# mfigura/Resilient-consensus-based-MARL

Measured on AMD Instinct MI355X. Metric: agent-steps/sec (whole RPBCAC training loop; + consensus-updates/sec), higher is better.
Workload: dtype f32 (matrix-core operands as 2 x f16 pieces: each fp32 operand to <= 1 ulp; the 20-unit layers run 3 of the 4 piece products)

## Files before the change

include/rcmarl.h:

```cpp
#ifndef RCMARL_H
#define RCMARL_H

#ifdef __cplusplus
extern "C" {
#endif

#define RCMARL_OK 0
#define RCMARL_ERR_ARG 1
#define RCMARL_ERR_LAUNCH 2
#define RCMARL_ERR_UNSUPPORTED 3

int rcmarl_abi_version(void);
int rcmarl_mb_job_layout(int what);
int rcmarl_fit_partial_size(int hid);
int rcmarl_actor_partial_size(int hid, int n_actions);
int rcmarl_rows_per_chunk(void);

int rcmarl_consensus_params(const float* msg, float* theta, const int* nbr, const int* coop, int S, int N,
                            int ldp, int P_hid, int d, int H, float* lo_dbg, float* hi_dbg, void* stream);
int rcmarl_consensus_params_circulant_supported(int N, int d, int H);
int rcmarl_consensus_params_circulant(const float* msg, float* theta, const int* coop, int S, int N, int ldp, int P_hid,
                                      int d, int H, float* lo_dbg, float* hi_dbg, void* stream);

typedef struct rcmarl_ragged_class {
// ... 28 lines not shown
                           void* stream);
int rcmarl_lattice_pack_dz_rowsum(const float* dz, void* dzp, float* sums, int sums_ld, int sums_off, int S, int N, int B, int hid,
                                  int ldb, int dzp_rt, int dzp_kt, void* stream);
int rcmarl_layer1_forward_lattice(const void* kp, int kp_rt, int kp_kt, const void* wp, int wp_rt, int wp_kt,
                                  const float* theta, float* a1t, int S, int N, int B, int in_dim, int hid, int ldp,
                                  int ldb, void* stream);
int rcmarl_layer1_backward_sgd_lattice(const void* ktp, int ktp_rt, int ktp_kt, const void* dzp, int dzp_rt, int dzp_kt,
                                       const float* alpha, float* theta, const int* mask, int S, int N, int B,
                                       int in_dim, int hid, int ldp, float lr, void* wp_out, int wp_rt, int wp_kt,
                                       void* stream);
int rcmarl_layer1_backward_sgd_lattice_tiled(const void* ktp, int ktp_rt, int ktp_kt, const void* dzp, int dzp_rt, int dzp_kt,
                                             const float* alpha, float* theta, const int* mask, int S, int N, int B,
                                             int in_dim, int hid, int ldp, float lr, void* wp_out, int wp_rt, int wp_kt,
                                             float* w_tiled, long w_tiled_bytes, int src_tiled, int dst_tiled, void* stream);
long rcmarl_lattice_w1_tiled_bytes(int S, int N, int in_dim, int hid);
int rcmarl_mid_fit_lattice(const float* a1t, const float* theta, const float* y, float* partials, void* dzp, int dzp_rt,
                           int dzp_kt, int S, int N, int B, int in_dim, int hid, int ldp, int ldb, int* ovf_flags, void* stream);


int rcmarl_shuffle_perms(const void* seeds, const int* calls, int n, int epochs, int B, int* perm, int S, void* stream);

int rcmarl_small_sgd(const float* partials, float* theta, const int* mask, float* loss_out, int S, int N,
                     int B, int in_dim, int hid, int ldp, float lr, void* stream);
int rcmarl_mid_value(const float* a1t, const float* theta, const float* r_applied, float gamma, float* out, int S,
                     int N, int B, int in_dim, int hid, int ldp, int ldb, void* stream);
int rcmarl_mid_value_f32(const float* a1t, const float* theta, const float* r_applied, float gamma, float* out, int S,
                         int N, int B, int in_dim, int hid, int ldp, int ldb, void* stream);

int rcmarl_consensus_head(const float* a1t, const float* theta, const float* msg, const int* nbr,
                          const int* coop, float* partials, float* agg_out, int S, int N, int B, int in_dim,
                          int hid, int ldp, int ldb, int d, int H, void* stream);
int rcmarl_consensus_head_ragged(const float* a1t, const float* theta, const float* msg, const int* nbr_off,
                                 const int* nbr_idx, const int* order, const rcmarl_ragged_class* classes, int n_classes,
                                 float* partials, float* agg_out, int S, int N, int B, int in_dim, int hid, int ldp, int ldb,
                                 void* stream);
int rcmarl_projection_residual(const float* a1t, const float* theta, const float* agg, const int* coop,
                               float* partials, int S, int N, int B, int in_dim, int hid, int ldp, int ldb,
                               void* stream);
int rcmarl_head_apply(const float* partials, float* theta, const int* coop, int S, int N, int B, int in_dim,
                      int hid, int ldp, void* stream);

int rcmarl_mid_actor(float* a1t, const float* theta, const float* act_t, const float* delta, float* partials, int S,
                     int N, int B, int in_dim, int hid, int n_actions, int ldp, int ldb, void* stream);
int rcmarl_small_adam(const float* partials, float* theta, float* adam_m, float* adam_v, const int* mask,
                      float* loss_out, int S, int N, int B, int in_dim, int hid, int n_actions, int ldp, float alpha,
                      float one_m_b1, float one_m_b2, float eps, void* stream);
// ... 164 lines not shown
```

resilient-consensus-based-marl_amd/capi.py:

```python
import ctypes as C
import os

c_f32p = C.c_void_p
c_i32p = C.c_void_p
c_u8p = C.c_void_p


class MbJob(C.Structure):
    _fields_ = [("x", C.c_void_p), ("x_seed_stride", C.c_long), ("theta", C.c_void_p), ("agents", C.c_void_p), ("n_adv", C.c_int),
                ("in_dim", C.c_int), ("ldp", C.c_int), ("reserved_", C.c_int), ("y", C.c_void_p), ("perm", C.c_void_p),
                ("loss_out", C.c_void_p), ("ovf_flags", C.c_void_p)]


class RaggedClass(C.Structure):
    _fields_ = [("d", C.c_int), ("H", C.c_int), ("first", C.c_int), ("count", C.c_int)]


c_f64p = C.c_void_p
c_stream = C.c_void_p

c_long = C.c_long
c_int = C.c_int
c_float = C.c_float

# ... 24 lines not shown
    "rcmarl_layer1_forward": [c_f32p, c_long, c_f32p, c_f32p, c_int, c_int, c_int, c_int, c_int, c_int, c_int,
                              c_stream],
    "rcmarl_layer1_backward_sgd": [c_f32p, c_long, c_f32p, c_f32p, c_u8p, c_int, c_int, c_int, c_int, c_int, c_int,
                                   c_int, c_float, c_stream],
    "rcmarl_layer1_backward_adam": [c_f32p, c_long, c_f32p, c_f32p, c_f32p, c_f32p, c_u8p, c_int, c_int, c_int, c_int,
                                    c_int, c_int, c_int, c_float, c_float, c_float, c_float, c_stream],
    "rcmarl_mid_fit": [c_f32p, c_f32p, c_f32p, c_f32p, c_int, c_int, c_int, c_int, c_int, c_int, c_int, c_stream],
    "rcmarl_lattice_encode": [c_f32p, c_long, c_f32p, c_int, c_int, c_int, c_u8p, c_int, c_int, c_u8p, c_int, c_int,
                              c_i32p, c_stream],
    "rcmarl_w1_split": [c_f32p, c_f32p, c_u8p, c_int, c_int, c_int, c_int, c_int, c_int, c_int, c_stream],
    "rcmarl_lattice_pack_dz": [c_f32p, c_u8p, c_int, c_int, c_int, c_int, c_int, c_int, c_int, c_stream],
    "rcmarl_lattice_pack_dz_rowsum": [c_f32p, c_u8p, c_f32p, c_int, c_int, c_int, c_int, c_int, c_int, c_int, c_int, c_int, c_stream],
    "rcmarl_layer1_forward_lattice": [c_u8p, c_int, c_int, c_u8p, c_int, c_int, c_f32p, c_f32p, c_int, c_int, c_int,
                                      c_int, c_int, c_int, c_int, c_stream],
    "rcmarl_layer1_backward_sgd_lattice": [c_u8p, c_int, c_int, c_u8p, c_int, c_int, c_f32p, c_f32p, c_u8p, c_int,
                                           c_int, c_int, c_int, c_int, c_int, c_float, c_u8p, c_int, c_int, c_stream],
    "rcmarl_layer1_backward_sgd_lattice_tiled": [c_u8p, c_int, c_int, c_u8p, c_int, c_int, c_f32p, c_f32p, c_u8p, c_int,
                                                 c_int, c_int, c_int, c_int, c_int, c_float, c_u8p, c_int, c_int, c_f32p, c_long,
                                                 c_int, c_int, c_stream],
    "rcmarl_mid_fit_lattice": [c_f32p, c_f32p, c_f32p, c_f32p, c_u8p, c_int, c_int, c_int, c_int, c_int, c_int, c_int,
                               c_int, c_int, c_i32p, c_stream],
    "rcmarl_shuffle_perms": [C.c_void_p, c_i32p, c_int, c_int, c_int, c_i32p, c_int, c_stream],
    "rcmarl_small_sgd": [c_f32p, c_f32p, c_u8p, c_f32p, c_int, c_int, c_int, c_int, c_int, c_int, c_float, c_stream],
    "rcmarl_mid_value": [c_f32p, c_f32p, c_f32p, c_float, c_f32p, c_int, c_int, c_int, c_int, c_int, c_int, c_int,
                         c_stream],
    "rcmarl_mid_value_f32": [c_f32p, c_f32p, c_f32p, c_float, c_f32p, c_int, c_int, c_int, c_int, c_int, c_int, c_int,
                             c_stream],
    "rcmarl_consensus_head": [c_f32p, c_f32p, c_f32p, c_i32p, c_u8p, c_f32p, c_f32p, c_int, c_int, c_int, c_int, c_int,
                              c_int, c_int, c_int, c_int, c_stream],
    "rcmarl_head_apply": [c_f32p, c_f32p, c_u8p, c_int, c_int, c_int, c_int, c_int, c_int, c_stream],
    "rcmarl_mid_actor": [c_f32p, c_f32p, c_f32p, c_f32p, c_f32p, c_int, c_int, c_int, c_int, c_int, c_int, c_int,
                         c_int, c_stream],
    "rcmarl_small_adam": [c_f32p, c_f32p, c_f32p, c_f32p, c_u8p, c_f32p, c_int, c_int, c_int, c_int, c_int, c_int,
                          c_int, c_float, c_float, c_float, c_float, c_stream],
    "rcmarl_team_reward": [c_f32p, c_long, c_u8p, c_int, c_f32p, c_int, c_int, c_int, c_int, c_stream],
    "rcmarl_projection_residual": [c_f32p, c_f32p, c_f32p, c_i32p, c_f32p, c_int, c_int, c_int, c_int, c_int, c_int,
                                   c_int, c_stream],
    "rcmarl_minibatch_fit": [c_f32p, c_long, c_f32p, c_i32p, c_int, c_f32p, c_i32p, c_int, c_int, c_int, c_int, c_int,
                             c_int, c_int, c_int, c_int, c_float, c_f32p, c_i32p, c_stream],
    "rcmarl_minibatch_actor": [c_f32p, c_long, c_f32p, c_f32p, c_f32p, c_i32p, c_int, c_f32p, c_f32p, c_i32p, c_int,
                               c_int, c_int, c_int, c_int, c_int, c_int, c_int, c_int, c_int, C.c_double, C.c_double,
                               C.c_double, C.c_double, c_int, c_f32p, c_stream],
    "rcmarl_minibatch_actor_wide_supported": [c_int, c_int, c_int, c_int],
    "rcmarl_minibatch_actor_wide": [c_f32p, c_long, c_f32p, c_f32p, c_f32p, c_f32p, c_i32p, c_int, c_f32p, c_f32p, c_i32p, c_int,
                                    c_int, c_int, c_int, c_int, c_int, c_int, c_int, c_int, c_int, C.c_double, C.c_double,
                                    C.c_double, C.c_double, c_int, c_f32p, c_stream],
# ... 145 lines not shown
```

resilient-consensus-based-marl_amd/csrc/lattice_gemm.hip:

```cpp
#include "rcmarl_lattice.h"
#include "rcmarl_lat_mainloop.h"
#include <type_traits>
#include <stdlib.h>

namespace {

__device__ __forceinline__ unsigned pack2(unsigned lo, unsigned hi) { return (lo & 0xffffu) | (hi << 16); }

__global__ __launch_bounds__(256) void k_lattice_encode(const float* __restrict__ x, long x_seed_stride,
                                                        const float* __restrict__ alpha, int B, int in_dim,
                                                        unsigned char* __restrict__ kp, int kp_rt, int kp_kt,
                                                        unsigned char* __restrict__ ktp, int ktp_rt, int ktp_kt,
                                                        int* __restrict__ flag, int kp_f16, int ktp_f16) {
  __shared__ unsigned short tileB[32][128 + 2], tileH[32][128 + 2];
  const int s = blockIdx.z, b0 = blockIdx.y * 32, c0 = blockIdx.x * 128;
  const int t = threadIdx.x;
  {
    const int cl = t & 127, c = c0 + cl;
    const float al = c < in_dim ? alpha[c] : 1.f;
    bool bad = false;
#pragma unroll 4
    for (int i = 0; i < 16; ++i) {
      const int bl = (t >> 7) + 2 * i, b = b0 + bl;
      float kq = 0.f;
// ... 160 lines not shown

struct LatPkOut {
  unsigned char* a1_bk; int bk_rt;
  unsigned char* a1_kb; int kb_kt;
  unsigned* s1; int s1_ld;
  int* ovf;
};

template <bool W8, bool F16, bool PK = false>
__global__ RC_LAT_OCC(W8 ? 512 : 256, W8 ? 4 : 2)
void k_lat_forward(const unsigned char* __restrict__ wp, int wp_rt, int wp_kt, const unsigned char* __restrict__ kp, int kp_rt,
                   int kp_kt, const float* __restrict__ theta, float* __restrict__ a1t, int S, int N, int B, int in_dim, int ldp,
                   int ldb, int mtiles, int ntiles, int hid, const LatPkOut pk) {
  constexpr int PA = F16 ? 2 : 3, PB = 1, MT = 2, NT = W8 ? 2 : 4, WM = 2, WN = W8 ? 4 : 2;
  typedef LatCfg<PA, PB, MT, NT, WM, WN> C;
  RCMARL_DYN_SMEM(unsigned char, lds);
  int s, w;
  lat_decode(blockIdx.x, mtiles * ntiles, S, s, w);
  const int bn = w % ntiles, bm = w / ntiles;
  LatOperands op;
  op.a = wp + (long)s * wp_rt * wp_kt * (PA * RC_PK_BLOCK); op.a_kt = wp_kt; op.art0 = bm * C::ART;
  op.b = kp + (long)s * kp_rt * kp_kt * (PB * RC_PK_BLOCK); op.b_kt = kp_kt; op.brt0 = bn * C::BRT;
  rc_f32x16 acc[MT][NT];
  lat_mainloop<PA, PB, MT, NT, WM, WN, false, F16>(op, (in_dim + 31) >> 5, lds, acc);
  const int ncols = N * hid;
  const float* theta_s = theta + (long)s * N * ldp;
  float* a1t_s = a1t + (long)s * ncols * ldb;
  __syncthreads();
  float* bias = reinterpret_cast<float*>(lds);
  if (threadIdx.x < C::BM) {
    const int col = bm * C::BM + threadIdx.x;
    const int ag = col / hid;
    bias[threadIdx.x] = col < ncols ? theta_s[(long)ag * ldp + in_dim * hid + (col - ag * hid)] : 0.f;
  }
  __syncthreads();
  const int lane = threadIdx.x & 63, half = lane >> 5;
  const int wave = __builtin_amdgcn_readfirstlane((int)(threadIdx.x >> 6)), wm = wave / WN, wn = wave % WN;
  float bv[MT][16];
#pragma unroll
  for (int mt = 0; mt < MT; ++mt)
#pragma unroll
    for (int q = 0; q < 4; ++q) {
      const float4 b4 = *reinterpret_cast<const float4*>(bias + wm * 32 * MT + 32 * mt + 8 * q + 4 * half);
      bv[mt][4 * q] = b4.x; bv[mt][4 * q + 1] = b4.y; bv[mt][4 * q + 2] = b4.z; bv[mt][4 * q + 3] = b4.w;
    }
  if constexpr (PK) {
    static_assert(F16, "packed activations exist in the two-piece f16 form");
// ... 428 lines not shown
```

resilient-consensus-based-marl_amd/csrc/mid_kernels.hip:

```cpp
#include "rcmarl_lattice.h"
#include <stdlib.h>
#include "selnet_generated.inc"

namespace {

constexpr bool kMidDropLL = true;

constexpr int ROWS = 256;
constexpr int LDR = ROWS + 1;

template <int HID> struct FitPart {
  static constexpr int gW2 = 0, gb2 = HID * HID, gW3 = gb2 + HID, gb3 = gW3 + HID, gb1 = gb3 + 1, loss = gb1 + HID,
                       SIZE = loss + 1, NSMALL = SIZE - gb2;
};
template <int HID, int A> struct ActorPart {
  static constexpr int gW2 = 0, gW3 = HID * HID, gb2 = gW3 + HID * A, gb3 = gb2 + HID, gb1 = gb3 + A,
                       loss = gb1 + HID, SIZE = loss + 1, NSMALL = SIZE - gb2;
};

template <int HID>
__device__ __forceinline__ void load_a1(const float* __restrict__ a1t, long row0, int ldb, int b, bool valid,
                                        float (&a1)[HID]) {
#pragma unroll
  for (int j = 0; j < HID; ++j) a1[j] = valid ? a1t[(row0 + j) * ldb + b] : 0.f;
// ... 541 lines not shown
#pragma unroll
        for (int u = 0; u < LU; ++u) {
          sRec[PT::gb1 + v8_unit(half, u)] = sm[u];
          sRec[PT::gW3 + v8_unit(half, u)] = sm[LU + u];
        }
        if (half == 0) { sRec[PT::gb3] = sm[2 * LU]; sRec[PT::loss] = sm[2 * LU + 1]; }
      }
    }
  }
  __syncthreads();
  if (amax > RC_V8_RANGE) ovf_flags[s * N + i] = ovf_gen;
  {
    const float* r0 = reinterpret_cast<const float*>(sPn + 0 * PANEL_B + 2 * PLANE * 2);
    const float* r1 = reinterpret_cast<const float*>(sPn + 1 * PANEL_B + 2 * PLANE * 2);
    const float* r2 = reinterpret_cast<const float*>(sPn + 2 * PANEL_B + 2 * PLANE * 2);
    const float* r3 = reinterpret_cast<const float*>(sPn + 3 * PANEL_B + 2 * PLANE * 2);
    float* out = partials + (((long)s * N + i) * gridDim.x + blockIdx.x) * PT::SIZE;
    out[r] = (r0[r] + r1[r]) + (r2[r] + r3[r]);
    if (r + ROWS < PT::SIZE) out[r + ROWS] = (r0[r + ROWS] + r1[r + ROWS]) + (r2[r + ROWS] + r3[r + ROWS]);
  }
}

template <int HID>
__global__ __launch_bounds__(256) void k_small_sgd(const float* __restrict__ partials, float* __restrict__ theta,
                                                   const int* __restrict__ mask,
                                                   float* __restrict__ loss_out, int N, int B, int in_dim, int ldp,
                                                   int nchunk, float lr) {
  typedef FitPart<HID> PT;
  const int s = blockIdx.y, i = blockIdx.x;
  if (mask && !mask[i]) return;
  const NetGeom g = make_geom(in_dim, HID, 1);
  float* th = theta + ((long)s * N + i) * ldp;
  const float* pp = partials + ((long)s * N + i) * nchunk * PT::SIZE;
  for (int e = threadIdx.x; e < PT::SIZE; e += blockDim.x) {
    float sum = 0.f;
    for (int c = 0; c < nchunk; ++c) sum += pp[(long)c * PT::SIZE + e];
    if (e == PT::loss) {
      if (loss_out) loss_out[(long)s * N + i] = sum / (float)B;
      continue;
    }
    int o;
    if (e < PT::gb2) o = g.o_W2 + e;
    else if (e < PT::gW3) o = g.o_b2 + (e - PT::gb2);
    else if (e < PT::gb3) o = g.o_W3 + (e - PT::gW3);
    else if (e < PT::gb1) o = g.o_b3;
    else o = g.o_b1 + (e - PT::gb1);
    th[o] = th[o] - lr * sum;
  }
}

template <int HID>
__global__ __launch_bounds__(256) void k_mid_value(const float* __restrict__ a1t, const float* __restrict__ theta,
                                                   const float* __restrict__ r_applied, float gamma,
                                                   float* __restrict__ out, int N, int B, int in_dim, int ldp,
                                                   int ldb) {
  const int s = blockIdx.z, i = blockIdx.y;
  const int b = blockIdx.x * ROWS + threadIdx.x;
  const bool valid = b < B;
  const NetGeom g = make_geom(in_dim, HID, 1);
  const float* th = theta + ((long)s * N + i) * ldp;
  float a1[HID], a2[HID];
  load_a1<HID>(a1t, ((long)s * N + i) * HID, ldb, b, valid, a1);
  layer2<HID>(th, g, a1, a2);
  const float v = head1<HID>(th + g.o_W3, th[g.o_b3], a2);
  if (valid) {
    const long o = ((long)s * N + i) * ldb + b;
    out[o] = r_applied ? r_applied[o] + gamma * v : v;
  }
}

// ... 761 lines not shown
  const dim3 grid(rc_ceil_div(nchunk, cpw), N, S), block(ROWS);
  rc_form_set(dzp, (rc_lat_f16_mode() >> 1) & 1);
  if (midfit_v8() && ovf_flags != nullptr) {
    int* flags = ovf_flags;
    int* gen = ovf_flags + (size_t)S * N;
    RCMARL_LAUNCH(k_bump_generation, dim3(1), dim3(1), 0, stream, gen);
    RC_HID_SWITCH(hid, RCMARL_LAUNCH((k_mid_fit_v8<HID_, true>), grid, block, 0, stream, const_cast<float*>(a1t), theta, y,
                                     partials, N, B, in_dim, ldp, ldb, nchunk, cpw, (unsigned char*)dzp, dzp_rt, dzp_kt, flags, (const int*)gen));
    RC_HID_SWITCH(hid, RCMARL_LAUNCH((k_mid_fit_v5<HID_, true, true>), grid, block, 0, stream, const_cast<float*>(a1t), theta, y,
                                     partials, N, B, in_dim, ldp, ldb, nchunk, cpw, (unsigned char*)dzp, dzp_rt, dzp_kt,
                                     (const int*)flags, (const int*)gen));
  } else if (rc_lat_f16_mode() & 2) {
    RC_HID_SWITCH(hid, RCMARL_LAUNCH((k_mid_fit_v5<HID_, true, true>), grid, block, 0, stream, const_cast<float*>(a1t), theta, y,
                                     partials, N, B, in_dim, ldp, ldb, nchunk, cpw, (unsigned char*)dzp, dzp_rt, dzp_kt,
                                     (const int*)nullptr, (const int*)nullptr));
  } else {
    RC_HID_SWITCH(hid, RCMARL_LAUNCH((k_mid_fit_v5<HID_, true>), grid, block, 0, stream, const_cast<float*>(a1t), theta, y,
                                     partials, N, B, in_dim, ldp, ldb, nchunk, cpw, (unsigned char*)dzp, dzp_rt, dzp_kt,
                                     (const int*)nullptr, (const int*)nullptr));
  }
  return rcmarl_check_launch();
}

RCMARL_EXPORT int rcmarl_small_sgd(const float* partials, float* theta, const int* mask, float* loss_out,
                                   int S, int N, int B, int in_dim, int hid, int ldp, float lr, void* stream) {
  if (!partials || !theta || S <= 0 || N <= 0 || B <= 0) return RCMARL_ERR_ARG;
  const int nchunk = rc_ceil_div(B, ROWS), nrec = rc_ceil_div(nchunk, midfit_cpw(nchunk, (long)S * N));
  const dim3 grid(N, S), block(256);
  RC_HID_SWITCH(hid, RCMARL_LAUNCH((k_small_sgd<HID_>), grid, block, 0, stream, partials, theta, mask, loss_out, N, B,
                                   in_dim, ldp, nrec, lr));
  return rcmarl_check_launch();
}

static int mid_value_impl(const float* a1t, const float* theta, const float* r_applied, float gamma, float* out, int S, int N, int B,
                          int in_dim, int hid, int ldp, int ldb, void* stream, bool f32_only) {
  if (bad_mid(a1t, theta, S, N, B, in_dim, hid, ldp, ldb) || !out) return RCMARL_ERR_ARG;
  const dim3 grid(rc_ceil_div(B, ROWS), N, S), block(ROWS);
  const char* mxe = getenv("RCMARL_MIDVALUE_MX");
  if (!f32_only && hid == 20 && !(mxe && atoi(mxe) == 0) && rc_lat_f16_mode() != 0) {
    const int nchunk = rc_ceil_div(B, ROWS);
    const long pairs = (long)N * S;
    int wgs = pairs >= 2048 ? 2 : (pairs >= 512 ? 4 : nchunk);
    if (wgs * 32 < nchunk) wgs = (nchunk + 31) / 32;
    const int cpw = (nchunk + wgs - 1) / wgs;
    const dim3 gmx((unsigned)((nchunk + cpw - 1) / cpw), N, S);
    RCMARL_LAUNCH((k_mid_value_mx<20>), gmx, block, 0, stream, a1t, theta, r_applied, gamma, out, N, B, in_dim, ldp, ldb, nchunk, cpw);
    return rcmarl_check_launch();
  }
  RC_HID_SWITCH(hid, RCMARL_LAUNCH((k_mid_value<HID_>), grid, block, 0, stream, a1t, theta, r_applied, gamma, out, N,
                                   B, in_dim, ldp, ldb));
  return rcmarl_check_launch();
}

RCMARL_EXPORT int rcmarl_mid_value(const float* a1t, const float* theta, const float* r_applied, float gamma,
// ... 178 lines not shown
```

resilient-consensus-based-marl_amd/csrc/rcmarl_lat_mainloop.h:

```cpp
#pragma once
#include "rcmarl_lattice.h"

namespace {

__device__ __forceinline__ uint4 ld_u4(const unsigned char* p) { return *reinterpret_cast<const uint4*>(p); }
__device__ __forceinline__ void st_u4(unsigned char* p, const uint4& v) { *reinterpret_cast<uint4*>(p) = v; }

template <int PA, int PB, int MT, int NT, int WM = 2, int WN = 2> struct LatCfg {
  static constexpr int BM = 32 * MT * WM, BN = 32 * NT * WN, NWV = WM * WN;
  static_assert(BM % 128 == 0 && BN % 128 == 0, "block tile sides are multiples of 128");
  static constexpr int ART = BM / 128, BRT = BN / 128;
  static constexpr int A_KB = ART * PA * 8, B_KB = BRT * PB * 8;
  static constexpr int STAGE_KB = A_KB + B_KB, STAGE_BYTES = STAGE_KB * 1024;
  static constexpr int GLDS = STAGE_KB / NWV;
  static_assert(STAGE_KB % NWV == 0, "stage splits evenly over the wavefronts");
};

struct LatOperands {
  const unsigned char* a; const unsigned char* b;
  int a_kt, b_kt;
  int art0, brt0;
};

template <int PA, int PB, int MT, int NT, int WM, int WN, bool SPREAD, bool F16, bool DROP_LL = false>
__device__ __forceinline__ void lat_mainloop(const LatOperands& op, int n_ktiles, unsigned char* lds,
                                             rc_f32x16 (&acc)[MT][NT]) {
  typedef LatCfg<PA, PB, MT, NT, WM, WN> C;
  const int lane = threadIdx.x & 63;
  const int wave = __builtin_amdgcn_readfirstlane((int)(threadIdx.x >> 6));
  const int wm = wave / WN, wn = wave % WN;
  const int l31 = lane & 31, half = lane >> 5;
#pragma unroll
  for (int mt = 0; mt < MT; ++mt)
#pragma unroll
    for (int nt = 0; nt < NT; ++nt)
#pragma unroll
      for (int i = 0; i < 16; ++i) acc[mt][nt][i] = 0.f;

  const unsigned char* gsrc[C::GLDS];
  int gstep[C::GLDS];
#pragma unroll
  for (int i = 0; i < C::GLDS; ++i) {
    const int q = wave + C::NWV * i;
    if (q < C::A_KB) {
      const int seg = q / (PA * 8), off = q - seg * (PA * 8);
      gsrc[i] = op.a + ((long)(op.art0 + seg) * op.a_kt) * (PA * RC_PK_BLOCK) + off * 1024;
      gstep[i] = PA * RC_PK_BLOCK;
    } else {
      const int q2 = q - C::A_KB;
      const int seg = q2 / (PB * 8), off = q2 - seg * (PB * 8);
      gsrc[i] = op.b + ((long)(op.brt0 + seg) * op.b_kt) * (PB * RC_PK_BLOCK) + off * 1024;
      gstep[i] = PB * RC_PK_BLOCK;
    }
  }
  const unsigned lane16 = lane * 16;
  const rc_lds_t lds0 = rc_lds_addr(lds) + wave * 1024;
  auto stage = [&](int buf, int t) {
    const rc_lds_t dst = lds0 + buf * C::STAGE_BYTES;
#pragma unroll
    for (int i = 0; i < C::GLDS; ++i) RC_GLDS16S(gsrc[i] + (long)t * gstep[i], lane16, dst + i * (C::NWV * 1024));
  };
  auto stage_one = [&](int buf, int t, int i) {
    RC_GLDS16S(gsrc[i] + (long)t * gstep[i], lane16, lds0 + buf * C::STAGE_BYTES + i * (C::NWV * 1024));
  };
  static_assert(!DROP_LL || (PA == 2 && PB == 2 && !SPREAD), "DROP_LL: two pieces on both sides, plain issue order");
  constexpr int N_MFMA = 2 * PA * PB * MT * NT;
  constexpr int EVERY = (N_MFMA / 2) / C::GLDS > 0 ? (N_MFMA / 2) / C::GLDS : 1;
  static_assert(!SPREAD || EVERY * C::GLDS <= N_MFMA, "spread issue: every burst has a slot");

  const int sw = (l31 >> 2) & 3;
  const int co0 = ((0 + half) ^ sw) << 4, co1 = ((2 + half) ^ sw) << 4;
  int offA[MT], offB[NT];
#pragma unroll
  for (int mt = 0; mt < MT; ++mt) {
    const int row = wm * 32 * MT + 32 * mt + l31;
    offA[mt] = (row >> 7) * PA * RC_PK_BLOCK + (row & 127) * 64;
  }
#pragma unroll
  for (int nt = 0; nt < NT; ++nt) {
    const int row = wn * 32 * NT + 32 * nt + l31;
    offB[nt] = C::A_KB * 1024 + (row >> 7) * PB * RC_PK_BLOCK + (row & 127) * 64;
  }

  stage(0, 0);
  for (int t = 0; t < n_ktiles; ++t) {
    const int cur = t & 1;
    RC_WAIT_VMEM();
    __syncthreads();
    const bool more = t + 1 < n_ktiles;
    if (more && !SPREAD) stage(cur ^ 1, t + 1);
    const unsigned char* st = lds + cur * C::STAGE_BYTES;
#pragma unroll
    for (int ks = 0; ks < 2; ++ks) {
      const int co = ks == 0 ? co0 : co1;
      uint4 af[MT][PA], bf[NT][PB];
#pragma unroll
      for (int mt = 0; mt < MT; ++mt)
#pragma unroll
        for (int p = 0; p < PA; ++p) af[mt][p] = ld_u4(st + offA[mt] + p * RC_PK_BLOCK + co);
#pragma unroll
      for (int nt = 0; nt < NT; ++nt)
#pragma unroll
        for (int p = 0; p < PB; ++p) bf[nt][p] = ld_u4(st + offB[nt] + p * RC_PK_BLOCK + co);
#pragma unroll
      for (int pa = PA - 1; pa >= 0; --pa)
#pragma unroll
        for (int pb = PB - 1; pb >= 0; --pb) {
          if (DROP_LL && pa == PA - 1 && pb == PB - 1) continue;
#pragma unroll
          for (int mt = 0; mt < MT; ++mt)
#pragma unroll
            for (int nt = 0; nt < NT; ++nt) {
              acc[mt][nt] = F16 ? rc_mfma_f16(af[mt][pa], bf[nt][pb], acc[mt][nt]) : rc_mfma_bf16(af[mt][pa], bf[nt][pb], acc[mt][nt]);
// ... 73 lines not shown
```

resilient-consensus-based-marl_amd/engine.py:

```python
import contextlib
import gc
import math
import os
import time

import numpy as np
import torch

from . import capi
from . import lattice as LT

HID = 20
COOP, FAULTY, GREEDY, MALICIOUS = "Cooperative", "Faulty", "Greedy", "Malicious"
W1_TILED_AUTO = True


def pad64(n):
    return (int(n) + 63) // 64 * 64


def net_numel(in_dim, out_dim, hid=HID):
    return in_dim * hid + hid + hid * hid + hid + hid * out_dim + out_dim


def net_shapes(in_dim, out_dim, hid=HID):
    return [(in_dim, hid), (hid,), (hid, hid), (hid,), (hid, out_dim), (out_dim,)]


def flatten_params(params):
    return np.concatenate([np.asarray(p, dtype=np.float32).ravel() for p in params])


def unflatten_params(vec, in_dim, out_dim, hid=HID):
    out, o = [], 0
    for sh in net_shapes(in_dim, out_dim, hid):
        n = int(np.prod(sh))
        out.append(np.array(vec[o:o + n], dtype=np.float32).reshape(sh))
        o += n
    return out


class EngineConfig:

    def __init__(self, n_agents, agent_label, in_nodes, H=0, gamma=0.9, slow_lr=0.002, fast_lr=0.01, n_actions=5,
                 n_states=2, max_ep_len=20, n_ep_fixed=50, n_epochs=10, buffer_size=2000, common_reward=False,
                 nrow=5, ncol=5, n_seeds=1, rng_mode="device", mu=0.1, scaling=True, randomize_state=True,
                 local_fit_steps=5, lattice="auto", critic_hid=HID, actor_hid=HID, tr_hid=HID, adv_wide2="auto",
                 w1_tiled="auto"):
        self.n_agents, self.agent_label = int(n_agents), list(agent_label)
        self.in_nodes = [list(map(int, row)) for row in in_nodes]
        self.gamma, self.slow_lr, self.fast_lr = float(gamma), float(slow_lr), float(fast_lr)
        self.n_actions, self.n_states = int(n_actions), int(n_states)
        self.max_ep_len, self.n_ep_fixed, self.n_epochs = int(max_ep_len), int(n_ep_fixed), int(n_epochs)
        self.buffer_size, self.common_reward = int(buffer_size), bool(common_reward)
        self.nrow, self.ncol, self.n_seeds = int(nrow), int(ncol), int(n_seeds)
        self.rng_mode, self.mu, self.scaling, self.randomize_state = rng_mode, float(mu), bool(scaling), bool(randomize_state)
        self.local_fit_steps = int(local_fit_steps)
        self.lattice = lattice
        self.critic_hid = int(critic_hid)
        self.actor_hid = int(actor_hid)
        self.tr_hid = int(tr_hid)
        if not any(adv_wide2 is v for v in (True, False)) and adv_wide2 != "auto":
            raise ValueError("adv_wide2 must be 'auto', True or False")
        self.adv_wide2 = adv_wide2
        if not any(w1_tiled is v for v in (True, False)) and w1_tiled != "auto":
            raise ValueError("w1_tiled must be 'auto', True or False")
        self.w1_tiled = w1_tiled
        assert len(self.agent_label) == self.n_agents and len(self.in_nodes) == self.n_agents
        if np.ndim(H) == 0:
            self.H_per_agent = [int(H)] * self.n_agents
        else:
            self.H_per_agent = [int(h) for h in H]
            if len(self.H_per_agent) != self.n_agents:
                raise ValueError("H must be an int or one int per agent (got %d for %d agents)" % (len(self.H_per_agent), self.n_agents))
        self.degrees = [len(row) for row in self.in_nodes]
        for i, row in enumerate(self.in_nodes):
            if not row or row[0] != i:
                raise ValueError("in_nodes[i][0] must be i (own value first, agents/resilient_CAC_agents.py:49)")
            if any(j < 0 or j >= self.n_agents for j in row):
                raise ValueError("in_nodes[%d] names an agent outside 0..%d" % (i, self.n_agents - 1))
            if self.agent_label[i] == COOP and (self.H_per_agent[i] < 0 or len(row) < 2 * self.H_per_agent[i] + 1):
                raise ValueError("need d >= 2H+1 (agent %d: d = %d, H = %d)" % (i, len(row), self.H_per_agent[i]))
        self.regular = len(set(self.degrees)) == 1 and len(set(self.H_per_agent)) == 1
        self.H = self.H_per_agent[0] if self.regular else max([h for h, l in zip(self.H_per_agent, self.agent_label) if l == COOP],
                                                               default=max(self.H_per_agent))
        if self.n_states != 2 or self.n_actions != 5:
            raise ValueError("the grid-world has 2 state dims and 5 actions per agent")
        if rng_mode not in ("device", "numpy"):
            raise ValueError("rng_mode must be 'device' or 'numpy'")
        for lab in self.agent_label:
# ... 909 lines not shown
        if self._sharded(net):
            y, mask = self._wv(y), self._wv(mask)
            with self._agent_window():
                return self._local_fit(net, xkey, y, B, mask, partials)
        if self.hid[net] != HID:
            return self._local_fit_wide(net, xkey, y, B, mask)
        L, S, N = self.lib, self.S, self.N
        msg = self.msg[net]
        if self._fit_as_chains(net, mask):
            ptr, stride = self._x(xkey)
            L.rcmarl_minibatch_fit(ptr, stride, msg.data_ptr(), self.coop_idx.data_ptr(), self.n_coop, y.data_ptr(), None, S, N, B,
                                   self.in_dim[net], HID, self.ldp[net], self.ldb, B, self.cfg.local_fit_steps, self.cfg.fast_lr,
                                   self.loss[net].data_ptr(), self.ovf_flags(("chain", net), S * max(self.n_coop, 1)).data_ptr(),
                                   self.stream)
            self.a1_cached[net] = False
            return
        a1 = self.a1net[net]
        ptr, stride = self._x(xkey)
        lat = self._lattice_ok(xkey, B, 0) and xkey in self.lat_ktp
        g = self.lat_geom[xkey] if lat else None
        dzp, wp = (self.lat_dzp_f[xkey], self.lat_wp_f[xkey]) if lat else (None, None)
        partials = self.partials if partials is None else partials
        wp_fresh = False
        for step in range(self.cfg.local_fit_steps):
            if not (step == 0 and self.a1_cached[net]):
                self._layer1(xkey, msg, net, B, buf=a1, wp_fresh=wp_fresh)
            if lat:
                L.rcmarl_mid_fit_lattice(a1.data_ptr(), msg.data_ptr(), y.data_ptr(), partials.data_ptr(),
                                         dzp.data_ptr(), g.dzp[0], g.dzp[1], S, N, B, self.in_dim[net], HID,
                                         self.ldp[net], self.ldb, self.ovf_flags(("mid", net), S * N + 1).data_ptr(), self.stream)
            else:
                L.rcmarl_mid_fit(a1.data_ptr(), msg.data_ptr(), y.data_ptr(), partials.data_ptr(), S, N, B,
                                 self.in_dim[net], HID, self.ldp[net], self.ldb, self.stream)
            L.rcmarl_small_sgd(partials.data_ptr(), msg.data_ptr(), mask.data_ptr(),
                               self.loss[net].data_ptr() if step == 0 else None, S, N, B, self.in_dim[net], HID,
                               self.ldp[net], self.cfg.fast_lr, self.stream)
            if lat:
                last = step == self.cfg.local_fit_steps - 1
                args = (self.lat_ktp[xkey].data_ptr(), g.ktp[0], g.ktp[1], dzp.data_ptr(), g.dzp[0], g.dzp[1],
                        self.lat_alpha[xkey].data_ptr(), msg.data_ptr(), mask.data_ptr(), S, N, B, self.in_dim[net], HID,
                        self.ldp[net], self.cfg.fast_lr, None if last else wp.data_ptr(), g.wp[0], g.wp[1])
                wt = self.lat_w1_tiled
                if wt is not None and self.cfg.local_fit_steps >= 2:
                    L.rcmarl_layer1_backward_sgd_lattice_tiled(*args, wt.data_ptr(), 4 * wt.numel(), int(step > 0), int(not last),
                                                               self.stream)
                else:
                    L.rcmarl_layer1_backward_sgd_lattice(*args, self.stream)
                wp_fresh = True
            else:
                L.rcmarl_layer1_backward_sgd(ptr, stride, a1.data_ptr(), msg.data_ptr(), mask.data_ptr(), S, N, B,
                                             self.in_dim[net], HID, self.ldp[net], self.ldb, self.cfg.fast_lr, self.stream)
        self.a1_cached[net] = False

    def ovf_flags(self, key, n):
        d = self.__dict__.setdefault("_ovf_flags", {})
        t = d.get(key)
        if t is None or t.numel() < n:
            t = d[key] = torch.zeros(int(n), dtype=torch.int32, device=self.dev)
        return t

    def _fit_as_chains(self, net, mask):
        if self.hid[net] != HID or self.in_dim[net] > 20 or self.lat_active or mask is not self.coop or self.n_coop == 0:
            return False
        if self.dev.type != "cuda" and os.environ.get("RCMARL_FIT_CHAINS") != "1":
            return False
        e = os.environ.get("RCMARL_FIT_CHAINS")
        if e is not None:
            return e not in ("0", "false")
        return self.S * self.n_coop >= 1024

    def _value(self, xkey, theta, net, out, B, row0=0, r_applied=None, scratch=None, gather=False, value_f32=False):
        if self._sharded(net) and scratch is None:
            th, o, r = self._wv(theta), self._wv(out), self._wv(r_applied)
            with self._agent_window():
                self._value(xkey, th, net, o, B, row0, r, value_f32=value_f32)
# ... 11 lines not shown
    def _k1(self, net, g_hid):
        L, c = self.lib, self.cfg
        if self._windowed:
            sc = self.shard.sc[net]
            assert g_hid == sc.P_hid
            sc.stream = self.stream
            sc.exchange(self.msg[net])
            sc.consensus()
            sc.gather(self.theta[net])
            return
        if not c.regular:
            if self.classes:
                L.rcmarl_consensus_params_ragged(self.msg[net].data_ptr(), self.theta[net].data_ptr(), self.nbr_off.data_ptr(),
                                                 self.nbr_idx.data_ptr(), self.order.data_ptr(), self.class_table, len(self.classes),
                                                 self.S, self.N, self.ldp[net], g_hid, None, None, self.stream)
        elif self.k1_circulant:
            L.rcmarl_consensus_params_circulant(self.msg[net].data_ptr(), self.theta[net].data_ptr(), self.coop.data_ptr(),
                                                self.S, self.N, self.ldp[net], g_hid, c.d, c.H, None, None, self.stream)
        else:
            L.rcmarl_consensus_params(self.msg[net].data_ptr(), self.theta[net].data_ptr(), self.nbr.data_ptr(),
                                      self.coop.data_ptr(), self.S, self.N, self.ldp[net], g_hid, c.d, c.H, None, None,
                                      self.stream)

    def _cached_rows_ok(self, net, row0, nrows):
        ep = self.cfg.max_ep_len
        return (self.td_shortcut and self.a1_cached[net] and self.rows_episode_aligned and self.hid[net] == HID and ep >= 2
                and row0 % ep == 0 and nrows % ep == 0)

    def _value_cached(self, net, out, row0, nrows, r_applied=None):
        if self._sharded(net):
            o, r = self._wv(out), self._wv(r_applied)
            with self._agent_window():
                self._value_cached(net, o, row0, nrows, r)
            return self._allgather_rows(out, 0, nrows)
        self.lib.rcmarl_mid_value(self.a1net[net].data_ptr() + 4 * row0, self.theta[net].data_ptr(), self._p(r_applied),
                                  self.cfg.gamma, out.data_ptr(), self.S, self.N, nrows, self.in_dim[net], HID,
                                  self.ldp[net], self.ldb, self.stream)

    def _value_next_cached(self, out, row0, nrows, r_applied, scratch):
        c, L, S, N = self.cfg, self.lib, self.S, self.N
        ep, th = c.max_ep_len, self.theta["critic"]
        L.rcmarl_mid_value(self.a1net["critic"].data_ptr() + 4 * (row0 + 1), th.data_ptr(), self._p(r_applied), c.gamma,
                           out.data_ptr(), S, N, nrows - 1, self.in_c, HID, self.ldp["critic"], self.ldb, self.stream)
        nt = nrows // ep
        ns_w = self.rp["ns"].shape[2]
        if self._ns_term is None or self._ns_term.numel() < S * nt * ns_w:
            self._ns_term = torch.empty(S * nt * ns_w, dtype=torch.float32, device=self.dev)
        ns_term = self._ns_term
        nptr, nstride = self._x("ns", row0)
        L.rcmarl_gather_rows(nptr, nstride, ep - 1, ep, nt, ns_w, ns_term.data_ptr(), S, self.stream)
# ... 82 lines not shown
                                               self.nbr_idx.data_ptr(), self.order.data_ptr(), self.class_table, len(self.classes),
                                               self.partials.data_ptr(), None, S, N, B, self.in_dim[net], HID, self.ldp[net],
                                               self.ldb, self.stream)
        else:
            L.rcmarl_consensus_head(a1.data_ptr(), self.theta[net].data_ptr(), msg_all.data_ptr(),
                                    self.nbr.data_ptr(), self.coop.data_ptr(), self.partials.data_ptr(), None, S, N, B,
                                    self.in_dim[net], HID, self.ldp[net], self.ldb, c.d, c.H, self.stream)
        self.a1_cached[net] = self.reuse_activations
        L.rcmarl_head_apply(self.partials.data_ptr(), self.theta[net].data_ptr(), self.coop.data_ptr(), S, N, B,
                            self.in_dim[net], HID, self.ldp[net], self.stream)

    def _timed(self, key, t0):
        if self.profile_phases:
            self.sync()
            t1 = time.perf_counter()
            self.timers[key] += t1 - t0
            return t1
        return t0

    profile_phases = False
    reuse_activations = True

    def _epoch_body(self, B, t0):
        if self.shard is not None and not self.shard.shard_tr:
            self.msg["tr"].copy_(self.theta["tr"])
        with self._agent_window():
            if self.shard is None or self.shard.shard_tr:
                self.msg["tr"].copy_(self.theta["tr"])
            self.msg["critic"].copy_(self.theta["critic"])
        self._td_target(B)
        join = self._adversary_messages_async(B)
        if self.dev.type == "cuda" and self._fit_as_chains("tr", self.coop) and self._fit_as_chains("critic", self.coop):
            if getattr(self, "chain_stream", None) is None:
                self.chain_stream = torch.cuda.Stream(device=self.dev)
            main = torch.cuda.current_stream(self.dev)
            fork = torch.cuda.Event()
            fork.record(main)
            self.chain_stream.wait_event(fork)
            with torch.cuda.stream(self.chain_stream):
                self._local_fit("tr", "sa", self.ybuf["r_fit"], B, self.coop)
                tr_done = torch.cuda.Event()
                tr_done.record(self.chain_stream)
            self._local_fit("critic", "s", self.ybuf["y_c"], B, self.coop)
            main.wait_event(tr_done)
        else:
            self._local_fit("tr", "sa", self.ybuf["r_fit"], B, self.coop)
            self._local_fit("critic", "s", self.ybuf["y_c"], B, self.coop)
        if join is not None:
            torch.cuda.current_stream(self.dev).wait_event(join)
        t0 = self._timed("phase1", t0)
        self._consensus("critic", "s", B)
        self._consensus("tr", "sa", B)
        return self._timed("phase2", t0)

    def _graph_wanted(self):
        e = os.environ.get("RCMARL_GRAPH")
        if e is not None:
            want = e not in ("0", "false")
        else:
            want = self.S * self.N <= 256
        if not want or self.dev.type != "cuda" or self.shard is not None or self.wide or self.profile_phases:
            return False
        if hasattr(self, "adv") and self.adv.fit and not self.adv._multi_ok() and \
                os.environ.get("RCMARL_ADV_ASYNC", "1") not in ("0", "false"):
            return False
        return not getattr(self.lib, "enabled", False)

    def _epoch(self, B, epoch, t0):
        if epoch == 0 or not self._graph_wanted() or not (self.a1_cached["critic"] and self.a1_cached["tr"]):
            return self._epoch_body(B, t0)
        key = (B, self.lat_active, bool(self.td_shortcut), bool(self.rows_episode_aligned), bool(self.k1_circulant), bool(self.cfg.regular),
               bool(self.reuse_activations), self.cap, self.lib.rcmarl_lattice_f16_mode(), os.environ.get("RCMARL_LAT_W8"),
               os.environ.get("RCMARL_MIDFIT"),
               bool(hasattr(self, "adv") and self.adv._multi_ok()), os.environ.get("RCMARL_ADV_ASYNC", "1"))
        g = self._graphs.get(key)
        if g is None:
            if len(self._graphs) >= 8:
                self._graphs.pop(next(iter(self._graphs)))
            g = torch.cuda.CUDAGraph()
            calls0 = list(self.adv.calls) if hasattr(self, "adv") else None
            gc_was_on = gc.isenabled()
            gc.collect()
            gc.disable()
            captured = False
            try:
                with torch.cuda.graph(g):
                    self._epoch_body(B, t0)
                captured = True
            finally:
                if gc_was_on:
                    gc.enable()
                if calls0 is not None:
                    g.rcmarl_draws = self.adv.calls[0] - calls0[0]
                    self.adv.calls = calls0
                    if self.adv.base_dev is not None:
                        try:
# ... 248 lines not shown
```

Before: 22.11 million.

## Fit first local step from live theta and skip dead wavefronts in lattice forward

Adds a small-SGD variant that reads parameters from one buffer and writes to another. The first local-fit step can then read theta directly, which removes the theta-to-msg copy at the start of each epoch. When the critic activations are not cached, the layer-1 forward for the TD target is computed up front so the fit can reuse it. Separately, wavefronts whose output columns lie past B skip the matrix instructions in the lattice mainloop. The cost is more gating conditions and extra CUDA graph key variants, and aliasing between theta and msg must stay correct.

```diff
diff --git a/include/rcmarl.h b/include/rcmarl.h
--- a/include/rcmarl.h
+++ b/include/rcmarl.h
@@ -74,6 +74,8 @@
 
 int rcmarl_small_sgd(const float* partials, float* theta, const int* mask, float* loss_out, int S, int N,
                      int B, int in_dim, int hid, int ldp, float lr, void* stream);
+int rcmarl_small_sgd_from(const float* partials, const float* src, float* dst, const int* mask, float* loss_out, int S, int N,
+                          int B, int in_dim, int hid, int ldp, float lr, void* stream);
 int rcmarl_mid_value(const float* a1t, const float* theta, const float* r_applied, float gamma, float* out, int S,
                      int N, int B, int in_dim, int hid, int ldp, int ldb, void* stream);
 int rcmarl_mid_value_f32(const float* a1t, const float* theta, const float* r_applied, float gamma, float* out, int S,
diff --git a/resilient-consensus-based-marl_amd/capi.py b/resilient-consensus-based-marl_amd/capi.py
--- a/resilient-consensus-based-marl_amd/capi.py
+++ b/resilient-consensus-based-marl_amd/capi.py
@@ -70,6 +70,7 @@
                                c_int, c_int, c_i32p, c_stream],
     "rcmarl_shuffle_perms": [C.c_void_p, c_i32p, c_int, c_int, c_int, c_i32p, c_int, c_stream],
     "rcmarl_small_sgd": [c_f32p, c_f32p, c_u8p, c_f32p, c_int, c_int, c_int, c_int, c_int, c_int, c_float, c_stream],
+    "rcmarl_small_sgd_from": [c_f32p, c_f32p, c_f32p, c_u8p, c_f32p, c_int, c_int, c_int, c_int, c_int, c_int, c_float, c_stream],
     "rcmarl_mid_value": [c_f32p, c_f32p, c_f32p, c_float, c_f32p, c_int, c_int, c_int, c_int, c_int, c_int, c_int,
                          c_stream],
     "rcmarl_mid_value_f32": [c_f32p, c_f32p, c_f32p, c_float, c_f32p, c_int, c_int, c_int, c_int, c_int, c_int, c_int,
diff --git a/resilient-consensus-based-marl_amd/csrc/lattice_gemm.hip b/resilient-consensus-based-marl_amd/csrc/lattice_gemm.hip
--- a/resilient-consensus-based-marl_amd/csrc/lattice_gemm.hip
+++ b/resilient-consensus-based-marl_amd/csrc/lattice_gemm.hip
@@ -206,7 +206,8 @@
   op.a = wp + (long)s * wp_rt * wp_kt * (PA * RC_PK_BLOCK); op.a_kt = wp_kt; op.art0 = bm * C::ART;
   op.b = kp + (long)s * kp_rt * kp_kt * (PB * RC_PK_BLOCK); op.b_kt = kp_kt; op.brt0 = bn * C::BRT;
   rc_f32x16 acc[MT][NT];
-  lat_mainloop<PA, PB, MT, NT, WM, WN, false, F16>(op, (in_dim + 31) >> 5, lds, acc);
+  const bool dead = !PK && bn * C::BN + __builtin_amdgcn_readfirstlane((int)(threadIdx.x >> 6)) % WN * (32 * NT) >= B;
+  lat_mainloop<PA, PB, MT, NT, WM, WN, false, F16, false, !PK>(op, (in_dim + 31) >> 5, lds, acc, dead);
   const int ncols = N * hid;
   const float* theta_s = theta + (long)s * N * ldp;
   float* a1t_s = a1t + (long)s * ncols * ldb;
diff --git a/resilient-consensus-based-marl_amd/csrc/mid_kernels.hip b/resilient-consensus-based-marl_amd/csrc/mid_kernels.hip
--- a/resilient-consensus-based-marl_amd/csrc/mid_kernels.hip
+++ b/resilient-consensus-based-marl_amd/csrc/mid_kernels.hip
@@ -587,7 +587,7 @@
 }
 
 template <int HID>
-__global__ __launch_bounds__(256) void k_small_sgd(const float* __restrict__ partials, float* __restrict__ theta,
+__global__ __launch_bounds__(256) void k_small_sgd(const float* __restrict__ partials, const float* src, float* dst,
                                                    const int* __restrict__ mask,
                                                    float* __restrict__ loss_out, int N, int B, int in_dim, int ldp,
                                                    int nchunk, float lr) {
@@ -595,7 +595,8 @@
   const int s = blockIdx.y, i = blockIdx.x;
   if (mask && !mask[i]) return;
   const NetGeom g = make_geom(in_dim, HID, 1);
-  float* th = theta + ((long)s * N + i) * ldp;
+  const float* th0 = src + ((long)s * N + i) * ldp;
+  float* th = dst + ((long)s * N + i) * ldp;
   const float* pp = partials + ((long)s * N + i) * nchunk * PT::SIZE;
   for (int e = threadIdx.x; e < PT::SIZE; e += blockDim.x) {
     float sum = 0.f;
@@ -610,7 +611,7 @@
     else if (e < PT::gb3) o = g.o_W3 + (e - PT::gW3);
     else if (e < PT::gb1) o = g.o_b3;
     else o = g.o_b1 + (e - PT::gb1);
-    th[o] = th[o] - lr * sum;
+    th[o] = th0[o] - lr * sum;
   }
 }
 
@@ -1418,14 +1419,19 @@
   return rcmarl_check_launch();
 }
 
+RCMARL_EXPORT int rcmarl_small_sgd_from(const float* partials, const float* src, float* dst, const int* mask, float* loss_out,
+                                        int S, int N, int B, int in_dim, int hid, int ldp, float lr, void* stream) {
+  if (!partials || !src || !dst || S <= 0 || N <= 0 || B <= 0) return RCMARL_ERR_ARG;
+  const int nchunk = rc_ceil_div(B, ROWS), nrec = rc_ceil_div(nchunk, midfit_cpw(nchunk, (long)S * N));
+  const dim3 grid(N, S), block(256);
+  RC_HID_SWITCH(hid, RCMARL_LAUNCH((k_small_sgd<HID_>), grid, block, 0, stream, partials, src, dst, mask, loss_out, N, B,
+                                   in_dim, ldp, nrec, lr));
+  return rcmarl_check_launch();
+}
+
 RCMARL_EXPORT int rcmarl_small_sgd(const float* partials, float* theta, const int* mask, float* loss_out,
                                    int S, int N, int B, int in_dim, int hid, int ldp, float lr, void* stream) {
-  if (!partials || !theta || S <= 0 || N <= 0 || B <= 0) return RCMARL_ERR_ARG;
-  const int nchunk = rc_ceil_div(B, ROWS), nrec = rc_ceil_div(nchunk, midfit_cpw(nchunk, (long)S * N));
-  const dim3 grid(N, S), block(256);
-  RC_HID_SWITCH(hid, RCMARL_LAUNCH((k_small_sgd<HID_>), grid, block, 0, stream, partials, theta, mask, loss_out, N, B,
-                                   in_dim, ldp, nrec, lr));
-  return rcmarl_check_launch();
+  return rcmarl_small_sgd_from(partials, theta, theta, mask, loss_out, S, N, B, in_dim, hid, ldp, lr, stream);
 }
 
 static int mid_value_impl(const float* a1t, const float* theta, const float* r_applied, float gamma, float* out, int S, int N, int B,
diff --git a/resilient-consensus-based-marl_amd/csrc/rcmarl_lat_mainloop.h b/resilient-consensus-based-marl_amd/csrc/rcmarl_lat_mainloop.h
--- a/resilient-consensus-based-marl_amd/csrc/rcmarl_lat_mainloop.h
+++ b/resilient-consensus-based-marl_amd/csrc/rcmarl_lat_mainloop.h
@@ -22,9 +22,9 @@
   int art0, brt0;
 };
 
-template <int PA, int PB, int MT, int NT, int WM, int WN, bool SPREAD, bool F16, bool DROP_LL = false>
+template <int PA, int PB, int MT, int NT, int WM, int WN, bool SPREAD, bool F16, bool DROP_LL = false, bool SKIP_DEAD = false>
 __device__ __forceinline__ void lat_mainloop(const LatOperands& op, int n_ktiles, unsigned char* lds,
-                                             rc_f32x16 (&acc)[MT][NT]) {
+                                             rc_f32x16 (&acc)[MT][NT], bool dead = false) {
   typedef LatCfg<PA, PB, MT, NT, WM, WN> C;
   const int lane = threadIdx.x & 63;
   const int wave = __builtin_amdgcn_readfirstlane((int)(threadIdx.x >> 6));
@@ -67,6 +67,7 @@
   constexpr int N_MFMA = 2 * PA * PB * MT * NT;
   constexpr int EVERY = (N_MFMA / 2) / C::GLDS > 0 ? (N_MFMA / 2) / C::GLDS : 1;
   static_assert(!SPREAD || EVERY * C::GLDS <= N_MFMA, "spread issue: every burst has a slot");
+  static_assert(!SKIP_DEAD || !SPREAD, "a dead wavefront's bursts are not tied to its matrix instructions");
 
   const int sw = (l31 >> 2) & 3;
   const int co0 = ((0 + half) ^ sw) << 4, co1 = ((2 + half) ^ sw) << 4;
@@ -89,6 +90,7 @@
     __syncthreads();
     const bool more = t + 1 < n_ktiles;
     if (more && !SPREAD) stage(cur ^ 1, t + 1);
+    if (SKIP_DEAD && dead) continue;
     const unsigned char* st = lds + cur * C::STAGE_BYTES;
 #pragma unroll
     for (int ks = 0; ks < 2; ++ks) {
diff --git a/resilient-consensus-based-marl_amd/engine.py b/resilient-consensus-based-marl_amd/engine.py
--- a/resilient-consensus-based-marl_amd/engine.py
+++ b/resilient-consensus-based-marl_amd/engine.py
@@ -13,6 +13,7 @@
 HID = 20
 COOP, FAULTY, GREEDY, MALICIOUS = "Cooperative", "Faulty", "Greedy", "Malicious"
 W1_TILED_AUTO = True
+FIT_FROM_LIVE_AUTO = True
 
 
 def pad64(n):
@@ -46,7 +47,7 @@
                  n_states=2, max_ep_len=20, n_ep_fixed=50, n_epochs=10, buffer_size=2000, common_reward=False,
                  nrow=5, ncol=5, n_seeds=1, rng_mode="device", mu=0.1, scaling=True, randomize_state=True,
                  local_fit_steps=5, lattice="auto", critic_hid=HID, actor_hid=HID, tr_hid=HID, adv_wide2="auto",
-                 w1_tiled="auto"):
+                 w1_tiled="auto", fit_from_live="auto"):
         self.n_agents, self.agent_label = int(n_agents), list(agent_label)
         self.in_nodes = [list(map(int, row)) for row in in_nodes]
         self.gamma, self.slow_lr, self.fast_lr = float(gamma), float(slow_lr), float(fast_lr)
@@ -66,6 +67,9 @@
         if not any(w1_tiled is v for v in (True, False)) and w1_tiled != "auto":
             raise ValueError("w1_tiled must be 'auto', True or False")
         self.w1_tiled = w1_tiled
+        if not any(fit_from_live is v for v in (True, False)) and fit_from_live != "auto":
+            raise ValueError("fit_from_live must be 'auto', True or False")
+        self.fit_from_live = fit_from_live
         assert len(self.agent_label) == self.n_agents and len(self.in_nodes) == self.n_agents
         if np.ndim(H) == 0:
             self.H_per_agent = [int(H)] * self.n_agents
@@ -1021,23 +1025,30 @@
         dzp, wp = (self.lat_dzp_f[xkey], self.lat_wp_f[xkey]) if lat else (None, None)
         partials = self.partials if partials is None else partials
         wp_fresh = False
+        live = self._fit_from_live(net, xkey, B, mask)
         for step in range(self.cfg.local_fit_steps):
+            src = self.theta[net] if live and step == 0 else msg
             if not (step == 0 and self.a1_cached[net]):
-                self._layer1(xkey, msg, net, B, buf=a1, wp_fresh=wp_fresh)
+                self._layer1(xkey, src, net, B, buf=a1, wp_fresh=wp_fresh)
             if lat:
-                L.rcmarl_mid_fit_lattice(a1.data_ptr(), msg.data_ptr(), y.data_ptr(), partials.data_ptr(),
+                L.rcmarl_mid_fit_lattice(a1.data_ptr(), src.data_ptr(), y.data_ptr(), partials.data_ptr(),
                                          dzp.data_ptr(), g.dzp[0], g.dzp[1], S, N, B, self.in_dim[net], HID,
                                          self.ldp[net], self.ldb, self.ovf_flags(("mid", net), S * N + 1).data_ptr(), self.stream)
             else:
                 L.rcmarl_mid_fit(a1.data_ptr(), msg.data_ptr(), y.data_ptr(), partials.data_ptr(), S, N, B,
                                  self.in_dim[net], HID, self.ldp[net], self.ldb, self.stream)
-            L.rcmarl_small_sgd(partials.data_ptr(), msg.data_ptr(), mask.data_ptr(),
-                               self.loss[net].data_ptr() if step == 0 else None, S, N, B, self.in_dim[net], HID,
-                               self.ldp[net], self.cfg.fast_lr, self.stream)
+            if src is msg:
+                L.rcmarl_small_sgd(partials.data_ptr(), msg.data_ptr(), mask.data_ptr(),
+                                   self.loss[net].data_ptr() if step == 0 else None, S, N, B, self.in_dim[net], HID,
+                                   self.ldp[net], self.cfg.fast_lr, self.stream)
+            else:
+                L.rcmarl_small_sgd_from(partials.data_ptr(), src.data_ptr(), msg.data_ptr(), mask.data_ptr(),
+                                        self.loss[net].data_ptr(), S, N, B, self.in_dim[net], HID, self.ldp[net],
+                                        self.cfg.fast_lr, self.stream)
             if lat:
                 last = step == self.cfg.local_fit_steps - 1
                 args = (self.lat_ktp[xkey].data_ptr(), g.ktp[0], g.ktp[1], dzp.data_ptr(), g.dzp[0], g.dzp[1],
-                        self.lat_alpha[xkey].data_ptr(), msg.data_ptr(), mask.data_ptr(), S, N, B, self.in_dim[net], HID,
+                        self.lat_alpha[xkey].data_ptr(), src.data_ptr(), mask.data_ptr(), S, N, B, self.in_dim[net], HID,
                         self.ldp[net], self.cfg.fast_lr, None if last else wp.data_ptr(), g.wp[0], g.wp[1])
                 wt = self.lat_w1_tiled
                 if wt is not None and self.cfg.local_fit_steps >= 2:
@@ -1050,6 +1061,14 @@
                 L.rcmarl_layer1_backward_sgd(ptr, stride, a1.data_ptr(), msg.data_ptr(), mask.data_ptr(), S, N, B,
                                              self.in_dim[net], HID, self.ldp[net], self.ldb, self.cfg.fast_lr, self.stream)
         self.a1_cached[net] = False
+
+    def _fit_from_live(self, net, xkey, B, mask):
+        want = FIT_FROM_LIVE_AUTO if self.cfg.fit_from_live == "auto" else self.cfg.fit_from_live
+        return bool(want and self.hid[net] == HID and self.shard is None and not self._windowed
+                    and mask is self.coop and self.n_coop == self.N
+                    and getattr(self, "lat_enabled", False) and self._lattice_ok(xkey, B, 0) and xkey in self.lat_ktp
+                    and self.lat_w1_tiled is not None and self.cfg.local_fit_steps >= 2
+                    and not self._fit_as_chains(net, mask))
 
     def ovf_flags(self, key, n):
         d = self.__dict__.setdefault("_ovf_flags", {})
@@ -1107,10 +1126,18 @@
                                       self.coop.data_ptr(), self.S, self.N, self.ldp[net], g_hid, c.d, c.H, None, None,
                                       self.stream)
 
-    def _cached_rows_ok(self, net, row0, nrows):
+    def _cached_rows_ok(self, net, row0, nrows, cached=None):
         ep = self.cfg.max_ep_len
-        return (self.td_shortcut and self.a1_cached[net] and self.rows_episode_aligned and self.hid[net] == HID and ep >= 2
+        cached = self.a1_cached[net] if cached is None else cached
+        return (self.td_shortcut and cached and self.rows_episode_aligned and self.hid[net] == HID and ep >= 2
                 and row0 % ep == 0 and nrows % ep == 0)
+
+    td_from_fit_forward = True
+
+    def _td_from_fit_forward(self, B):
+        return bool(self.td_from_fit_forward and self.reuse_activations and not self.a1_cached["critic"] and self.shard is None
+                    and getattr(self, "lat_enabled", False) and self._lattice_ok("s", B, 0) and "s" in self.lat_ktp
+                    and self._cached_rows_ok("critic", 0, B, cached=True))
 
     def _value_cached(self, net, out, row0, nrows, r_applied=None):
         if self._sharded(net):
@@ -1239,12 +1266,17 @@
     reuse_activations = True
 
     def _epoch_body(self, B, t0):
+        live = {"tr": self._fit_from_live("tr", "sa", B, self.coop), "critic": self._fit_from_live("critic", "s", B, self.coop)}
         if self.shard is not None and not self.shard.shard_tr:
             self.msg["tr"].copy_(self.theta["tr"])
         with self._agent_window():
-            if self.shard is None or self.shard.shard_tr:
+            if (self.shard is None or self.shard.shard_tr) and not live["tr"]:
                 self.msg["tr"].copy_(self.theta["tr"])
-            self.msg["critic"].copy_(self.theta["critic"])
+            if not live["critic"]:
+                self.msg["critic"].copy_(self.theta["critic"])
+        if self._td_from_fit_forward(B):
+            self._layer1("s", self.theta["critic"], "critic", B, buf=self.a1net["critic"])
+            self.a1_cached["critic"] = True
         self._td_target(B)
         join = self._adversary_messages_async(B)
         if self.dev.type == "cuda" and self._fit_as_chains("tr", self.coop) and self._fit_as_chains("critic", self.coop):
@@ -1289,6 +1321,7 @@
         key = (B, self.lat_active, bool(self.td_shortcut), bool(self.rows_episode_aligned), bool(self.k1_circulant), bool(self.cfg.regular),
                bool(self.reuse_activations), self.cap, self.lib.rcmarl_lattice_f16_mode(), os.environ.get("RCMARL_LAT_W8"),
                os.environ.get("RCMARL_MIDFIT"),
+               self._fit_from_live("tr", "sa", B, self.coop), self._fit_from_live("critic", "s", B, self.coop),
                bool(hasattr(self, "adv") and self.adv._multi_ok()), os.environ.get("RCMARL_ADV_ASYNC", "1"))
         g = self._graphs.get(key)
         if g is None:
```

Measured after the change: 22.34 million, median of 6. +1.1%, better.
